# CityU-AIM-Group/SCAN

Hardware: AMD Instinct MI355X
Metric: train images/sec (whole node), VGG16 C2F 1024x2048 (higher is better)
Workload: dtype f32 (fp32 storage, fp32 multiply, fp32 accumulate -- the reference's arithmetic; the convolutions run it on the bf16 matrix cores as bf16x6: every fp32 operand cut into 3 bf16 pieces = all 24 significand bits, 6 bf16 MFMAs per product)

## Files before the change

scan_amd/csrc/capi.cpp:

```cpp
#include <stdarg.h>
#include <stdio.h>
#include <string.h>

#include "../../include/scan_hip.h"
#include "conv_launch.h"

static thread_local char g_err[512] = "";

extern "C" void scan_set_error(const char* fmt, ...) {
  va_list ap;
  va_start(ap, fmt);
  vsnprintf(g_err, sizeof(g_err), fmt, ap);
  va_end(ap);
}

extern "C" const char* scan_last_error(void) { return g_err; }
extern "C" int scan_abi_version(void) { return 1; }

int g_scan_deterministic = 0;

struct Knob {
  const char* key;
  int* slot;
  int dflt;
};
static Knob* knob_table(int* count) {
  static Knob knobs[] = {
      {"conv_bn256", &g_scan_conv_bn256, 0},   {"conv_v2", &g_scan_conv_v2, 0},         {"conv_wg1024", &g_scan_conv_wg1024, 0},
      {"conv_w8", &g_scan_conv_w8, 0},         {"conv_tpb3", &g_scan_conv_tpb3, 0},     {"conv_bn64_th16", &g_scan_conv_bn64_th16, 0},
      {"conv_glds", &g_scan_conv_glds, 0},     {"wgrad_v6", &g_scan_wgrad_v6, 0},       {"wgrad_prio", &g_scan_wgrad_prio, 0},
      {"wgrad_tile", &g_scan_wgrad_tile, 0},   {"wgrad_wgs", &g_scan_wgrad_wgs, 0},     {"gconv_mfma", &g_scan_gconv_mfma, 0},
      {"dbscan_bf16x3", &g_scan_dbscan_bf16x3, 0}, {"reduce_blocks", &g_scan_reduce_blocks, 0}, {"conv1x1", &g_scan_conv1x1, 0},
      {"conv_wino", &g_scan_conv_wino, 0},     {"wgrad_wino", &g_scan_wgrad_wino, 0},   {"wino_tpb", &g_scan_wino_tpb, 0},
      {"deterministic", &g_scan_deterministic, 0}, {"dynconv_generic", &g_scan_dynconv_generic, 0},
  };
  static bool init = false;
  if (!init) {
    for (auto& k : knobs) k.dflt = *k.slot;
    init = true;
  }
  *count = (int)(sizeof(knobs) / sizeof(knobs[0]));
  return knobs;
}
static Knob* find_knob(const char* key) {
  int n = 0;
  Knob* t = knob_table(&n);
  if (key == nullptr) return nullptr;
  for (int i = 0; i < n; ++i)
    if (strcmp(key, t[i].key) == 0) return &t[i];
  return nullptr;
}

extern "C" int scan_tune(const char* key, int value) {
  Knob* k = find_knob(key);
  if (k == nullptr) return SCAN_TUNE_UNKNOWN;
  const int old = *k->slot;
  *k->slot = value;
  return old;
}

extern "C" int scan_tune_get(const char* key) {
  const Knob* k = find_knob(key);
  return k == nullptr ? SCAN_TUNE_UNKNOWN : *k->slot;
}

extern "C" int scan_tune_default(const char* key) {
  const Knob* k = find_knob(key);
  return k == nullptr ? SCAN_TUNE_UNKNOWN : k->dflt;
}

extern "C" const char* scan_tune_key(int index) {
  int n = 0;
  const Knob* t = knob_table(&n);
  return (index >= 0 && index < n) ? t[index].key : nullptr;
}
```

scan_amd/csrc/conv_launch.h:

```cpp
#pragma once
#include <hip/hip_runtime_api.h>
#include <stdint.h>

#include "../../include/scan_hip.h"

extern int g_scan_conv_v2;
extern int g_scan_conv_bn256, g_scan_conv_wg1024, g_scan_conv_w8, g_scan_conv_tpb3;
extern int g_scan_conv_glds, g_scan_conv_bn64_th16, g_scan_conv1x1;
extern int g_scan_conv_wino, g_scan_wino_tpb;
extern int g_scan_wgrad_v6, g_scan_wgrad_prio, g_scan_wgrad_tile, g_scan_wgrad_wgs, g_scan_wgrad_wino;
extern int g_scan_gconv_mfma;
extern int g_scan_dynconv_generic;
extern int g_scan_dbscan_bf16x3;
extern int g_scan_reduce_blocks;

struct ConvArgs {
  const float* x;
  const scan_pyramid_t* od;
  const scan_pyramid_t* sd;
  int32_t Cs;
  const __bf16* w[3];
  int32_t Csw;
  const float* bias;
  const float* mask;
  float* y;
  int32_t Nout, Ns, relu, map;
  hipStream_t st;
  double* gn_ws;
};

struct ConvInst {
  int id;
  void (*launch)(const ConvArgs&);
};
ConvInst pick3x3(int np, const scan_pyramid_t* d, int32_t Nout, bool whole_chunks);
ConvInst pick1x1(int np, const scan_pyramid_t* yd, int32_t Nout, int32_t Csw);
void conv3x3_wino_launch(const ConvArgs& a);

void gen1_conv3x3_launch(const ConvArgs& a);
void gen1_conv1x1_launch(const ConvArgs& a);

typedef scan_conv_wgrad_plan_t WgradPlan;
int wgrad_split_plan(const char* name, int np, int ksize, int stride, int32_t Cs, int32_t Cout, const scan_pyramid_t* d, WgradPlan* p);
int wgrad_split_run(const char* name, const WgradPlan& p, const float* x, const scan_pyramid_t* xd, int32_t Cs, const float* dy,
                    const scan_pyramid_t* yd, int32_t Cout, int32_t Cout_s, float* dw, float* db, int32_t accumulate, float* ws,
                    void* stream);
int wgrad_generic_plan(const char* name, int np, int ksize, int stride, int32_t Cs, int32_t Cout, const scan_pyramid_t* yd, WgradPlan* p);
int wgrad_generic_run(const char* name, const WgradPlan& p, const float* x, const scan_pyramid_t* xd, int32_t Cs, const float* dy,
                      const scan_pyramid_t* yd, int32_t Cout, int32_t Cout_s, float* dw, float* db, int32_t accumulate, float* ws,
                      void* stream);
```

scan_amd/csrc/gconv.hip:

```cpp
#include "common.h"

#define GC_G 128

template <int CTRL, int ROW_MASK>
__device__ __forceinline__ float dpp_add(float v) {
  const int r = __builtin_amdgcn_update_dpp(0, __builtin_bit_cast(int, v), CTRL, ROW_MASK, 0xF, false);
  return v + __builtin_bit_cast(float, r);
}
__device__ __forceinline__ float half_wave_sum_hi(float v) {
  v = dpp_add<0xB1, 0xF>(v);
  v = dpp_add<0x4E, 0xF>(v);
  v = dpp_add<0x141, 0xF>(v);
  v = dpp_add<0x140, 0xF>(v);
  v = dpp_add<0x142, 0xA>(v);
  return v;
}

__device__ __forceinline__ int64_t neighbour_row(const scan_pyramid_t& d, int64_t m, const RowCoord& rc, int oy, int ox) {
  const int y = rc.y + oy, x = rc.x + ox;
  if (y < 0 || y >= d.h[rc.lvl] || x < 0 || x >= d.w[rc.lvl]) return -1;
  return m + (int64_t)oy * d.w[rc.lvl] + ox;
}

__device__ __forceinline__ float4 zero4() { return make_float4(0.f, 0.f, 0.f, 0.f); }
// ... 237 lines not shown
    wv[t] = DO_DX ? *reinterpret_cast<const float4*>(w + ((int64_t)g * 9 + t) * GC + coff) : zero4();
    acc[t] = zero4();
  }
  const bool need_x = DO_DW || relu_mask;
  constexpr int UN = (DO_DX && DO_DW) ? 1 : GC_UNROLL;
  for (int64_t q0 = hw / G; q0 < M; q0 += UN * J) {
    float4 h[UN];
    float gy[UN][9];
#pragma unroll
    for (int u = 0; u < UN; ++u) {
      const int64_t q = q0 + u * J;
      h[u] = (q < M && need_x) ? *reinterpret_cast<const float4*>(x + q * GC + coff) : zero4();
      if (q < M) {
        const RowCoord rc = decode_row(d, q);
#pragma unroll
        for (int t = 0; t < 9; ++t) {
          const int64_t p = neighbour_row(d, q, rc, 1 - t / 3, 1 - t % 3);
          gy[u][t] = p >= 0 ? dy[p * Ns + g] : 0.f;
        }
      } else {
#pragma unroll
        for (int t = 0; t < 9; ++t) gy[u][t] = 0.f;
      }
    }
#pragma unroll
    for (int u = 0; u < UN; ++u) {
      const int64_t q = q0 + u * J;
      if (DO_DW) {
#pragma unroll
        for (int t = 0; t < 9; ++t) fma4(acc[t], gy[u][t], h[u]);
      }
      if (DO_DX && q < M) {
        float4 o = zero4();
#pragma unroll
        for (int t = 0; t < 9; ++t) fma4(o, gy[u][t], wv[t]);
        if (relu_mask) o = relu_mask4(h[u], o);
        *reinterpret_cast<float4*>(dx + q * GC + coff) = o;
      }
    }
  }
  if (!DO_DW) return;
  float* out = slab + (int64_t)hw * 9 * GC_G + 4 * l32;
#pragma unroll
  for (int t = 0; t < 9; ++t) *reinterpret_cast<float4*>(out + t * GC_G) = acc[t];
}

typedef float f32x4g __attribute__((ext_vector_type(4)));

__global__ __launch_bounds__(256) void gconv_taps_mfma_kernel(const float* __restrict__ x, int64_t M, int G, int GC,
                                                              const float* __restrict__ w, float* __restrict__ T,
                                                              uint32_t* __restrict__ relu_bits) {
  const int lane = threadIdx.x & 63;
  const int col = lane & 15, q = lane >> 4;
  const int64_t wave_id = (int64_t)blockIdx.x * 4 + (threadIdx.x >> 6);
  const int64_t n_waves = (int64_t)gridDim.x * 4;
  const int g = (int)(wave_id % G);
  float4 bw[8];
#pragma unroll
  for (int j = 0; j < 8; ++j)
    bw[j] = col < 9 ? *reinterpret_cast<const float4*>(w + ((int64_t)g * 9 + col) * GC + g * GC_G + 16 * j + 4 * q)
                    : make_float4(0.f, 0.f, 0.f, 0.f);
  const int64_t groups = (M + 15) / 16;
  for (int64_t gidx = wave_id / G; gidx < groups; gidx += n_waves / G) {
    const int64_t row = gidx * 16 + col;
    float4 av[8];
#pragma unroll
    for (int j = 0; j < 8; ++j)
      av[j] = row < M ? *reinterpret_cast<const float4*>(x + row * GC + g * GC_G + 16 * j + 4 * q)
                      : make_float4(0.f, 0.f, 0.f, 0.f);
    f32x4g acc = {0.f, 0.f, 0.f, 0.f};
    uint32_t bits = 0u;
#pragma unroll
    for (int j = 0; j < 8; ++j) {
      acc = __builtin_amdgcn_mfma_f32_16x16x4f32(av[j].x, bw[j].x, acc, 0, 0, 0);
      acc = __builtin_amdgcn_mfma_f32_16x16x4f32(av[j].y, bw[j].y, acc, 0, 0, 0);
      acc = __builtin_amdgcn_mfma_f32_16x16x4f32(av[j].z, bw[j].z, acc, 0, 0, 0);
      acc = __builtin_amdgcn_mfma_f32_16x16x4f32(av[j].w, bw[j].w, acc, 0, 0, 0);
      bits |= (av[j].x > 0.f ? 1u : 0u) << (4 * j) | (av[j].y > 0.f ? 2u : 0u) << (4 * j) |
              (av[j].z > 0.f ? 4u : 0u) << (4 * j) | (av[j].w > 0.f ? 8u : 0u) << (4 * j);
    }
    if (relu_bits != nullptr && row < M) relu_bits[(row * G + g) * 4 + q] = bits;
#pragma unroll
    for (int r = 0; r < 4; ++r) {
      const int64_t orow = gidx * 16 + 4 * q + r;
      if (col < 9 && orow < M) T[(orow * G + g) * 9 + col] = acc[r];
    }
  }
}

__global__ __launch_bounds__(256) void gconv_dx_mfma_kernel(const float* __restrict__ dy, int Ns, scan_pyramid_t d, int G,
                                                            int GC, const float* __restrict__ w,
                                                            const float* __restrict__ xmask,
                                                            const uint32_t* __restrict__ relu_bits,
                                                            float* __restrict__ dx) {
  const int64_t M = d.row_off[d.n_levels];
  const int lane = threadIdx.x & 63;
  const int col = lane & 15, q = lane >> 4;
  const int64_t wave_id = (int64_t)blockIdx.x * 4 + (threadIdx.x >> 6);
  const int64_t n_waves = (int64_t)gridDim.x * 4;
  const int g = (int)(wave_id % G);
  float aw[8][3];
#pragma unroll
  for (int tile = 0; tile < 8; ++tile)
#pragma unroll
    for (int s_ = 0; s_ < 3; ++s_) {
      const int t = 4 * s_ + q;
      aw[tile][s_] = t < 9 ? w[((int64_t)g * 9 + t) * GC + g * GC_G + 16 * tile + col] : 0.f;
    }
  const int64_t groups = (M + 15) / 16;
  for (int64_t gidx = wave_id / G; gidx < groups; gidx += n_waves / G) {
    const int64_t row = gidx * 16 + col;
    float gy[3] = {0.f, 0.f, 0.f};
    if (row < M) {
      const RowCoord rc = decode_row(d, row);
#pragma unroll
      for (int s_ = 0; s_ < 3; ++s_) {
        const int t = 4 * s_ + q;
        if (t < 9) {
          const int64_t p = neighbour_row(d, row, rc, 1 - t / 3, 1 - t % 3);
          if (p >= 0) gy[s_] = dy[p * Ns + g];
        }
      }
    }
    uint32_t bits = 0xffffffffu;
    float4 mk[8];
    if (relu_bits != nullptr) {
      if (row < M) bits = relu_bits[(row * G + g) * 4 + q];
    } else if (xmask != nullptr) {
#pragma unroll
      for (int tile = 0; tile < 8; ++tile)
        mk[tile] = row < M ? *reinterpret_cast<const float4*>(xmask + row * GC + g * GC_G + 16 * tile + 4 * q)
                           : make_float4(0.f, 0.f, 0.f, 0.f);
    }
#pragma unroll
    for (int tile = 0; tile < 8; ++tile) {
      f32x4g acc = {0.f, 0.f, 0.f, 0.f};
#pragma unroll
      for (int s_ = 0; s_ < 3; ++s_) acc = __builtin_amdgcn_mfma_f32_16x16x4f32(aw[tile][s_], gy[s_], acc, 0, 0, 0);
      float4 o = make_float4(acc[0], acc[1], acc[2], acc[3]);
      if (relu_bits != nullptr) {
        o.x = (bits >> (4 * tile + 0)) & 1u ? o.x : 0.f;
        o.y = (bits >> (4 * tile + 1)) & 1u ? o.y : 0.f;
        o.z = (bits >> (4 * tile + 2)) & 1u ? o.z : 0.f;
        o.w = (bits >> (4 * tile + 3)) & 1u ? o.w : 0.f;
      } else if (xmask != nullptr) {
        o = relu_mask4(mk[tile], o);
      }
      if (row < M) *reinterpret_cast<float4*>(dx + row * GC + g * GC_G + 16 * tile + 4 * q) = o;
    }
  }
}

__global__ __launch_bounds__(256) void gconv_slab_partial_kernel(const float* __restrict__ slab, int blocks, int n,
                                                                 int per_part, float* __restrict__ partial) {
  const int i = blockIdx.x * blockDim.x + threadIdx.x;
  if (i >= n) return;
  const int b0 = blockIdx.y * per_part;
  const int b1 = b0 + per_part < blocks ? b0 + per_part : blocks;
  float s = 0.f;
#pragma unroll 8
  for (int b = b0; b < b1; ++b) s += slab[(int64_t)b * n + i];
  partial[(int64_t)blockIdx.y * n + i] = s;
}

enum GconvDst {
  GC_DST_DW,
  GC_DST_DW_GENERIC,
  GC_DST_DE
};
template <GconvDst DST>
__device__ __forceinline__ int64_t gconv_dst_index(int i, int GC) {
  if (DST == GC_DST_DW_GENERIC) {
    const int gt = i / GC_G, c = i - gt * GC_G;
    return (int64_t)gt * GC + (gt / 9) * GC_G + c;
  }
  const int t = i / GC, c = i - t * GC;
  return DST == GC_DST_DW ? ((int64_t)(c / GC_G) * 9 + t) * GC + c : ((int64_t)(c / GC_G) * 9 + t) * GC_G + c % GC_G;
}

template <GconvDst DST>
__global__ __launch_bounds__(256) void gconv_reduce_kernel(const float* __restrict__ partial, int parts, int GC,
                                                           float* __restrict__ out, int accumulate) {
  const int i = blockIdx.x * blockDim.x + threadIdx.x;
  if (i >= 9 * GC) return;
  float s = 0.f;
  for (int b = 0; b < parts; ++b) s += partial[(int64_t)b * 9 * GC + i];
  float* dst = out + gconv_dst_index<DST>(i, GC);
  *dst = accumulate ? *dst + s : s;
}


__device__ __forceinline__ float4 act_hidden(float4 h, const float4 (&ev)[9], const float (&av)[9]) {
#pragma unroll
  for (int t = 0; t < 9; ++t) fma4(h, av[t], ev[t]);
  return relu_mask4(h, h);
}

#define GC_UNROLL_A 2
#define GC_PICK_UNI(G, kernel, ...) ((G) == 8 ? kernel<true, ##__VA_ARGS__> : kernel<false, ##__VA_ARGS__>)

template <bool UNI>
__global__ __launch_bounds__(256) void gconv_taps_act_kernel(const float* __restrict__ x, scan_pyramid_t d, int G, int GC,
                                                             const float* __restrict__ w, const float* __restrict__ a,
                                                             int lda, const float* __restrict__ E, float* __restrict__ T) {
  const int64_t M = d.row_off[d.n_levels];
  const int quads = GC >> 2, slots = 256 / quads;
  const int cq = threadIdx.x % quads, slot = threadIdx.x / quads;
  const int g = cq >> 5, l32 = cq & 31;
  float4 wv[9], ev[9];
#pragma unroll
  for (int t = 0; t < 9; ++t) {
    wv[t] = *reinterpret_cast<const float4*>(w + ((int64_t)g * 9 + t) * GC + 4 * cq);
    ev[t] = *reinterpret_cast<const float4*>(E + ((int64_t)g * 9 + t) * GC_G + 4 * l32);
  }
  const int64_t stride = (int64_t)gridDim.x * slots;
  for (int64_t q0 = (int64_t)blockIdx.x * slots + slot; q0 < M; q0 += GC_UNROLL_F * stride) {
    float4 h[GC_UNROLL_F];
#pragma unroll
    for (int u = 0; u < GC_UNROLL_F; ++u) {
      const int64_t q = q0 + u * stride;
      h[u] = q < M ? *reinterpret_cast<const float4*>(x + q * GC + 4 * cq) : zero4();
    }
#pragma unroll
    for (int u = 0; u < GC_UNROLL_F; ++u) {
      int64_t q = q0 + u * stride;
      if (UNI) q = uniform_row(q);
      if (q >= M) continue;
      float av[9];
      tap_values<1>(d, q, decode_row(d, q), a, lda, g, UNI, av);
      tap_store(T, q, G, g, l32, tap_sums(act_hidden(h[u], ev, av), wv, l32));
    }
  }
}

template <bool UNI, bool FUSE>
__global__ __launch_bounds__(256, (UNI && !FUSE) ? 3 : 2) void gconv_bwd_act_kernel(
    const float* __restrict__ x, const float* __restrict__ dy, int Ns, scan_pyramid_t d, int G, int GC,
    const float* __restrict__ w, const float* __restrict__ a, int lda, const float* __restrict__ E, float* __restrict__ dx,
    float* __restrict__ slab, float* __restrict__ T, float* __restrict__ slab_e) {
  __shared__ float red[9 * 1024];
  const int64_t M = d.row_off[d.n_levels];
  const int quads = GC >> 2, slots = 256 / quads;
  const int cq = threadIdx.x % quads, slot = threadIdx.x / quads;
  const int g = cq >> 5, l32 = cq & 31;
  float4 wv[9], ev[9], acc[9], acc_e[9];
#pragma unroll
  for (int t = 0; t < 9; ++t) {
    wv[t] = *reinterpret_cast<const float4*>(w + ((int64_t)g * 9 + t) * GC + 4 * cq);
    ev[t] = *reinterpret_cast<const float4*>(E + ((int64_t)g * 9 + t) * GC_G + 4 * l32);
    acc[t] = zero4();
    if (FUSE) acc_e[t] = zero4();
  }
  for (int64_t q0 = (int64_t)blockIdx.x * GC_UNROLL_A * slots + slot; q0 < M;
       q0 += (int64_t)gridDim.x * GC_UNROLL_A * slots) {
    float4 h[GC_UNROLL_A];
#pragma unroll
    for (int u = 0; u < GC_UNROLL_A; ++u) {
      const int64_t q = q0 + u * slots;
      h[u] = q < M ? *reinterpret_cast<const float4*>(x + q * GC + 4 * cq) : zero4();
    }
#pragma unroll
    for (int u = 0; u < GC_UNROLL_A; ++u) {
      int64_t q = q0 + u * slots;
      if (UNI) q = uniform_row(q);
      if (q >= M) continue;
      const RowCoord rc = decode_row(d, q);
      float av[9], gy[9];
      tap_values<1>(d, q, rc, a, lda, g, UNI, av);
      const float4 hv = act_hidden(h[u], ev, av);
      tap_values<-1>(d, q, rc, dy, Ns, g, UNI, gy);
      float4 o = zero4();
#pragma unroll
      for (int t = 0; t < 9; ++t) {
        fma4(acc[t], gy[t], hv);
        fma4(o, gy[t], wv[t]);
      }
      o = relu_mask4(hv, o);
      *reinterpret_cast<float4*>(dx + q * GC + 4 * cq) = o;
      if (FUSE) {
        float mine = 0.f;
#pragma unroll
        for (int t = 0; t < 9; ++t) {
          fma4(acc_e[t], av[t], o);
          const float s = half_wave_sum_hi(dot4(o, ev[8 - t]));
          if (l32 == 16 + t) mine = s;
        }
        tap_store(T, q, G, g, l32, mine);
      }
    }
  }
  slab_store(acc, red, slab, GC);
  if (FUSE) {
    __syncthreads();
    slab_store(acc_e, red, slab_e, GC);
  }
}

template <bool UNI>
__global__ __launch_bounds__(256) void gconv_act_grads_kernel(const float* __restrict__ dh, scan_pyramid_t d, int G, int GC,
                                                              const float* __restrict__ a, int lda,
                                                              const float* __restrict__ E, float* __restrict__ T,
                                                              float* __restrict__ slab) {
  __shared__ float red[9 * 1024];
  const int64_t M = d.row_off[d.n_levels];
  const int quads = GC >> 2, slots = 256 / quads;
  const int cq = threadIdx.x % quads, slot = threadIdx.x / quads;
  const int g = cq >> 5, l32 = cq & 31;
  float4 ev[9], acc[9];
#pragma unroll
  for (int t = 0; t < 9; ++t) {
    ev[t] = *reinterpret_cast<const float4*>(E + ((int64_t)g * 9 + t) * GC_G + 4 * l32);
    acc[t] = zero4();
  }
  for (int64_t q0 = (int64_t)blockIdx.x * GC_UNROLL_A * slots + slot; q0 < M;
       q0 += (int64_t)gridDim.x * GC_UNROLL_A * slots) {
    float4 h[GC_UNROLL_A];
#pragma unroll
    for (int u = 0; u < GC_UNROLL_A; ++u) {
      const int64_t q = q0 + u * slots;
      h[u] = q < M ? *reinterpret_cast<const float4*>(dh + q * GC + 4 * cq) : zero4();
    }
#pragma unroll
    for (int u = 0; u < GC_UNROLL_A; ++u) {
      int64_t q = q0 + u * slots;
      if (UNI) q = uniform_row(q);
      if (q >= M) continue;
      float av[9];
      tap_values<1>(d, q, decode_row(d, q), a, lda, g, UNI, av);
      float mine = 0.f;
#pragma unroll
      for (int t = 0; t < 9; ++t) {
        fma4(acc[t], av[t], h[u]);
        const float s = half_wave_sum_hi(dot4(h[u], ev[8 - t]));
        if (l32 == 16 + t) mine = s;
      }
      tap_store(T, q, G, g, l32, mine);
    }
  }
  slab_store(acc, red, slab, GC);
}

#define GC_MAX_BLOCKS 1024
#define GC_PARTS 32
#define GC_GMAX 31

static bool gconv_lane_mapped(int G) { return G == 1 || G == 2 || G == 4 || G == 8; }

static int gconv_check(const scan_pyramid_t* d, int G, int Cg, const char* who, bool any_g = false) {
  SCAN_CHECK_ARG(d && d->n_levels >= 1 && d->n_levels <= SCAN_MAX_LEVELS, "%s: bad pyramid", who);
  SCAN_CHECK_ARG(Cg == GC_G, "%s: only 128 channels per group are built (got %d)", who, Cg);
  if (any_g) {
    SCAN_CHECK_ARG(G >= 1 && G <= GC_GMAX, "%s: G=%d out of 1..%d", who, G, GC_GMAX);
    return 0;
  }
  SCAN_CHECK_ARG(gconv_lane_mapped(G), "%s: G=%d must be 1, 2, 4 or 8", who, G);
  return 0;
}

int g_scan_gconv_mfma = 0;

enum GconvFamily { GC_GENERIC, GC_FMA, GC_MFMA };
static GconvFamily gconv_family(int G, bool bits) {
  if (!gconv_lane_mapped(G)) return GC_GENERIC;
  return (g_scan_gconv_mfma || bits) ? GC_MFMA : GC_FMA;
}

extern "C" int32_t scan_gconv3x3_to1_max_groups(void) { return GC_GMAX; }

extern "C" int32_t scan_gconv3x3_to1_caps(int32_t G, int32_t Cg) {
  if (G < 1 || G > GC_GMAX || Cg != GC_G) return 0;
  const GconvFamily f = gconv_family(G, false);
  return SCAN_GCONV_RUNS | (f == GC_GENERIC ? 0 : SCAN_GCONV_LANE_MAPPED) | (f == GC_MFMA ? SCAN_GCONV_BITS : 0) |
         (f == GC_FMA ? SCAN_GCONV_ACT : 0);
}

struct GconvWs {
  int64_t slab, slab_e, total;
};
static GconvWs gconv_ws_layout(int64_t M, int G, int Cg, bool act) {
  const int64_t taps = M * G * 9, slab = (int64_t)(GC_MAX_BLOCKS + GC_PARTS) * 9 * G * Cg;
  if (act) return {taps, taps + slab, taps + 2 * slab};
  return {0, -1, taps > slab ? taps : slab};
}

extern "C" int64_t scan_gconv3x3_to1_ws_floats(const scan_pyramid_t* d, int32_t G, int32_t Cg) {
  return d ? gconv_ws_layout(d->row_off[d->n_levels], G, Cg, false).total : -1;
}

extern "C" int64_t scan_gconv3x3_to1_act_ws_floats(const scan_pyramid_t* d, int32_t G, int32_t Cg) {
  return d ? gconv_ws_layout(d->row_off[d->n_levels], G, Cg, true).total : -1;
}

static int gconv_generic_strides(int64_t M, int per, int max_j) {
  int64_t j = ((M + per - 1) / per + 7) / 8 * 8;
  if (j < 8) j = 8;
  if (j > max_j) j = max_j;
  return (int)j;
}

static int gconv_slab_blocks(int64_t M) {
  int64_t rpb = (M + GC_MAX_BLOCKS - 1) / GC_MAX_BLOCKS;
  if (rpb < 16) rpb = 16;
  return (int)((M + rpb - 1) / rpb);
}

static int gconv_wave_grid(int64_t M, int G) {
  int64_t tasks = ((M + 15) / 16) * G;
  int64_t blocks = (tasks + 3) / 4;
  if (blocks > 2048) blocks = 2048;
  if (blocks < 2) blocks = 2;
  return (int)((blocks + 1) / 2 * 2);
}

static int gconv_gather(const float* T, const scan_pyramid_t* d, int G, const float* bias, float* y, int ldy, int col0,
                        hipStream_t st) {
  const int64_t M = d->row_off[d->n_levels];
  hipLaunchKernelGGL(gconv_gather_kernel, dim3(grid_for(M * ldy, 256)), dim3(256), 0, st, T, *d, G, bias, y, ldy, col0);
  SCAN_LAUNCH_CHECK("gconv_gather");
  return 0;
}

template <GconvDst DST>
static int gconv_slab_to(float* slab, int blocks, int GC, float* out, int accumulate, hipStream_t st) {
  const int n = 9 * GC, per = (blocks + GC_PARTS - 1) / GC_PARTS, parts = (blocks + per - 1) / per;
  float* partial = slab + (int64_t)GC_MAX_BLOCKS * n;
  hipLaunchKernelGGL(gconv_slab_partial_kernel, dim3((n + 255) / 256, parts), dim3(256), 0, st, slab, blocks, n, per, partial);
  SCAN_LAUNCH_CHECK("gconv_slab_partial");
  hipLaunchKernelGGL(gconv_reduce_kernel<DST>, dim3((n + 255) / 256), dim3(256), 0, st, partial, parts, GC, out, accumulate);
  SCAN_LAUNCH_CHECK(DST == GC_DST_DE ? "gconv_act_reduce" : "gconv_wgrad_reduce");
  return 0;
}

static int gconv_forward(const float* x, const scan_pyramid_t* d, int G, int Cg, const float* w, const float* bias, float* y,
                         int Ns, float* ws, uint32_t* relu_bits, hipStream_t st, bool any_g = false) {
  if (gconv_check(d, G, Cg, "gconv3x3_to1_forward", any_g)) return -1;
  SCAN_CHECK_ARG(x && w && y && ws && Ns >= G, "gconv3x3_to1_forward: bad arguments (Ns=%d)", Ns);
  const int64_t M = d->row_off[d->n_levels];
  if (M == 0) return 0;
  const int GC = G * Cg;
  switch (gconv_family(G, relu_bits != nullptr)) {
    case GC_GENERIC:
      SCAN_CHECK_ARG(relu_bits == nullptr, "gconv3x3_to1_forward_bits: G=%d must be 1, 2, 4 or 8", G);
      hipLaunchKernelGGL(gconv_taps_generic_kernel, dim3(gconv_generic_strides(M, GC_UNROLL_F, 2048) / 8 * G), dim3(256), 0,
                         st, x, M, G, GC, w, ws);
      SCAN_LAUNCH_CHECK("gconv_taps_generic");
      break;
    case GC_MFMA:
      hipLaunchKernelGGL(gconv_taps_mfma_kernel, dim3(gconv_wave_grid(M, G)), dim3(256), 0, st, x, M, G, GC, w, ws, relu_bits);
      SCAN_LAUNCH_CHECK("gconv_taps");
      break;
    case GC_FMA: {
      const int slots = 256 / (GC / 4);
      hipLaunchKernelGGL(gconv_taps_kernel, dim3(grid_for((M + slots - 1) / slots, 1)), dim3(256), 0, st, x, M, G, GC, w, ws);
      SCAN_LAUNCH_CHECK("gconv_taps");
    }
  }
  return gconv_gather(ws, d, G, bias, y, Ns, 0, st);
}

template <bool DO_DX, bool DO_DW>
static void gconv_bwd_launch(bool generic, int grid, hipStream_t st, const float* x, const float* dy, int Ns,
                             const scan_pyramid_t* d, int G, int GC, const float* w, int relu_mask, float* dx, float* slab) {
  hipLaunchKernelGGL((generic ? gconv_bwd_generic_kernel<DO_DX, DO_DW> : gconv_bwd_kernel<DO_DX, DO_DW>), dim3(grid), dim3(256),
                     0, st, x, dy, Ns, *d, G, GC, w, relu_mask, dx, slab);
}

static int gconv_backward(const float* x, const float* dy, int Ns, const scan_pyramid_t* d, int G, int Cg, const float* w,
                          int relu_mask, const uint32_t* relu_bits, float* dx, float* dw, int accumulate, float* ws,
                          hipStream_t st, const char* who, bool any_g = false) {
  if (gconv_check(d, G, Cg, who, any_g)) return -1;
  SCAN_CHECK_ARG(dy && Ns >= G && (dx || dw), "%s: bad arguments (Ns=%d)", who, Ns);
  SCAN_CHECK_ARG(!dx || w, "%s: the data gradient needs the weights", who);
  SCAN_CHECK_ARG(!dw || (x && ws), "%s: the weight gradient needs x and a workspace", who);
  SCAN_CHECK_ARG(!(dx && relu_mask && !relu_bits) || x, "%s: the ReLU mask needs x or its bit mask", who);
  const int64_t M = d->row_off[d->n_levels];
  if (M == 0) return 0;
  const int GC = G * Cg;
  const GconvFamily family = gconv_family(G, relu_bits != nullptr);
  const bool generic = family == GC_GENERIC;
  SCAN_CHECK_ARG(!generic || relu_bits == nullptr, "%s: G=%d must be 1, 2, 4 or 8", who, G);
  const int blocks = generic ? gconv_generic_strides(M, 16, GC_MAX_BLOCKS) : gconv_slab_blocks(M);
  const int grid = generic ? blocks / 8 * G : blocks;
  float* slab = ws + gconv_ws_layout(M, G, Cg, false).slab;
  if (dx && family == GC_MFMA) {
    hipLaunchKernelGGL(gconv_dx_mfma_kernel, dim3(gconv_wave_grid(M, G)), dim3(256), 0, st, dy, Ns, *d, G, GC, w,
                       (relu_mask && !relu_bits) ? x : (const float*)nullptr, relu_bits, dx);
    SCAN_LAUNCH_CHECK(who);
    if (dw) gconv_bwd_launch<false, true>(generic, grid, st, x, dy, Ns, d, G, GC, w, 0, dx, slab);
  } else if (dx && dw) {
    gconv_bwd_launch<true, true>(generic, grid, st, x, dy, Ns, d, G, GC, w, relu_mask, dx, slab);
  } else if (dx) {
    gconv_bwd_launch<true, false>(generic, grid, st, x, dy, Ns, d, G, GC, w, relu_mask, dx, slab);
  } else {
    gconv_bwd_launch<false, true>(generic, grid, st, x, dy, Ns, d, G, GC, w, 0, dx, slab);
  }
  SCAN_LAUNCH_CHECK(who);
  if (!dw) return 0;
  return generic ? gconv_slab_to<GC_DST_DW_GENERIC>(slab, blocks, GC, dw, accumulate, st)
                 : gconv_slab_to<GC_DST_DW>(slab, blocks, GC, dw, accumulate, st);
}

extern "C" int scan_gconv3x3_to1_forward(const float* x, const scan_pyramid_t* d, int32_t G, int32_t Cg, const float* w,
                                         const float* bias, float* y, int32_t Ns, float* ws, void* stream) {
  return gconv_forward(x, d, G, Cg, w, bias, y, Ns, ws, nullptr, as_stream(stream));
}

extern "C" int scan_gconv3x3_to1_forward_bits(const float* x, const scan_pyramid_t* d, int32_t G, int32_t Cg,
                                              const float* w, const float* bias, float* y, int32_t Ns, float* ws,
                                              uint32_t* relu_bits, void* stream) {
  SCAN_CHECK_ARG(relu_bits, "gconv3x3_to1_forward_bits: null bit mask");
  return gconv_forward(x, d, G, Cg, w, bias, y, Ns, ws, relu_bits, as_stream(stream));
}

extern "C" int scan_gconv3x3_to1_dgrad(const float* dy, int32_t Ns, const scan_pyramid_t* d, int32_t G, int32_t Cg,
                                       const float* w, const float* mask, float* dx, void* stream) {
  SCAN_CHECK_ARG(dx, "gconv3x3_to1_dgrad: null output");
  return gconv_backward(mask, dy, Ns, d, G, Cg, w, mask != nullptr, nullptr, dx, nullptr, 0, nullptr, as_stream(stream),
                        "gconv3x3_to1_dgrad");
}

extern "C" int scan_gconv3x3_to1_wgrad(const float* x, const float* dy, int32_t Ns, const scan_pyramid_t* d, int32_t G,
                                       int32_t Cg, float* dw, int32_t accumulate, float* ws, void* stream) {
  SCAN_CHECK_ARG(dw, "gconv3x3_to1_wgrad: null output");
  return gconv_backward(x, dy, Ns, d, G, Cg, nullptr, 0, nullptr, nullptr, dw, accumulate, ws, as_stream(stream),
                        "gconv3x3_to1_wgrad");
}

extern "C" int scan_gconv3x3_to1_backward(const float* x, const float* dy, int32_t Ns, const scan_pyramid_t* d, int32_t G,
                                          int32_t Cg, const float* w, int32_t relu_mask, float* dx, float* dw,
                                          int32_t accumulate, float* ws, void* stream) {
  SCAN_CHECK_ARG(x && dx && dw, "gconv3x3_to1_backward: null pointer");
  return gconv_backward(x, dy, Ns, d, G, Cg, w, relu_mask, nullptr, dx, dw, accumulate, ws, as_stream(stream),
                        "gconv3x3_to1_backward");
}

extern "C" int scan_gconv3x3_to1_backward_bits(const float* x, const float* dy, int32_t Ns, const scan_pyramid_t* d,
                                               int32_t G, int32_t Cg, const float* w, const uint32_t* relu_bits, float* dx,
                                               float* dw, int32_t accumulate, float* ws, void* stream) {
  SCAN_CHECK_ARG(x && dx && dw && relu_bits, "gconv3x3_to1_backward_bits: null pointer");
  return gconv_backward(x, dy, Ns, d, G, Cg, w, 1, relu_bits, dx, dw, accumulate, ws, as_stream(stream),
                        "gconv3x3_to1_backward_bits");
}

extern "C" int scan_gconv3x3_to1_any_forward(const float* x, const scan_pyramid_t* d, int32_t G, int32_t Cg, const float* w,
                                             const float* bias, float* y, int32_t Ns, float* ws, void* stream) {
  return gconv_forward(x, d, G, Cg, w, bias, y, Ns, ws, nullptr, as_stream(stream), true);
}

extern "C" int scan_gconv3x3_to1_any_dgrad(const float* dy, int32_t Ns, const scan_pyramid_t* d, int32_t G, int32_t Cg,
                                           const float* w, const float* mask, float* dx, void* stream) {
  SCAN_CHECK_ARG(dx, "gconv3x3_to1_any_dgrad: null output");
  return gconv_backward(mask, dy, Ns, d, G, Cg, w, mask != nullptr, nullptr, dx, nullptr, 0, nullptr, as_stream(stream),
                        "gconv3x3_to1_any_dgrad", true);
}

extern "C" int scan_gconv3x3_to1_any_wgrad(const float* x, const float* dy, int32_t Ns, const scan_pyramid_t* d, int32_t G,
                                           int32_t Cg, float* dw, int32_t accumulate, float* ws, void* stream) {
  SCAN_CHECK_ARG(dw, "gconv3x3_to1_any_wgrad: null output");
  return gconv_backward(x, dy, Ns, d, G, Cg, nullptr, 0, nullptr, nullptr, dw, accumulate, ws, as_stream(stream),
                        "gconv3x3_to1_any_wgrad", true);
}

extern "C" int scan_gconv3x3_to1_any_backward(const float* x, const float* dy, int32_t Ns, const scan_pyramid_t* d, int32_t G,
                                              int32_t Cg, const float* w, int32_t relu_mask, float* dx, float* dw,
                                              int32_t accumulate, float* ws, void* stream) {
  SCAN_CHECK_ARG(x && dx && dw, "gconv3x3_to1_any_backward: null pointer");
  return gconv_backward(x, dy, Ns, d, G, Cg, w, relu_mask, nullptr, dx, dw, accumulate, ws, as_stream(stream),
                        "gconv3x3_to1_any_backward", true);
}

static int gconv_act_check(const scan_pyramid_t* d, int G, int Cg, const float* a, int lda, int a_col0, const float* E,
                           const char* who) {
  if (gconv_check(d, G, Cg, who)) return -1;
  SCAN_CHECK_ARG(a && E && a_col0 >= 0 && lda >= a_col0 + G, "%s: bad act map (lda=%d, first column %d, G=%d)", who, lda,
                 a_col0, G);
  return 0;
}

extern "C" int scan_gconv3x3_to1_act_forward(const float* x, const scan_pyramid_t* d, int32_t G, int32_t Cg, const float* w,
                                             const float* bias, const float* a, int32_t lda, int32_t a_col0, const float* E,
                                             float* y, int32_t Ns, float* ws, void* stream) {
  if (gconv_act_check(d, G, Cg, a, lda, a_col0, E, "gconv3x3_to1_act_forward")) return -1;
  SCAN_CHECK_ARG(x && w && y && ws && Ns >= G, "gconv3x3_to1_act_forward: bad arguments (Ns=%d)", Ns);
  const int64_t M = d->row_off[d->n_levels];
  if (M == 0) return 0;
  const int GC = G * Cg, slots = 256 / (GC / 4);
  hipStream_t st = as_stream(stream);
  hipLaunchKernelGGL(GC_PICK_UNI(G, gconv_taps_act_kernel), dim3(grid_for((M + slots - 1) / slots, 1)), dim3(256), 0, st, x, *d,
                     G, GC, w, a + a_col0, lda, E, ws);
  SCAN_LAUNCH_CHECK("gconv_taps_act");
  return gconv_gather(ws, d, G, bias, y, Ns, 0, st);
}

extern "C" int scan_gconv3x3_to1_act_backward(const float* x, const float* dy, int32_t Ns, const scan_pyramid_t* d, int32_t G,
                                              int32_t Cg, const float* w, const float* a, int32_t lda, int32_t a_col0,
                                              const float* E, float* dx, float* dw, int32_t accumulate, float* ws,
                                              void* stream) {
  if (gconv_act_check(d, G, Cg, a, lda, a_col0, E, "gconv3x3_to1_act_backward")) return -1;
  SCAN_CHECK_ARG(x && dy && w && dx && dw && ws && Ns >= G, "gconv3x3_to1_act_backward: bad arguments (Ns=%d)", Ns);
  const int64_t M = d->row_off[d->n_levels];
  if (M == 0) return 0;
  const int GC = G * Cg, blocks = gconv_slab_blocks(M);
  hipStream_t st = as_stream(stream);
  float* slab = ws + gconv_ws_layout(M, G, Cg, true).slab;
  hipLaunchKernelGGL(GC_PICK_UNI(G, gconv_bwd_act_kernel, false), dim3(blocks), dim3(256), 0, st, x, dy, Ns, *d, G, GC, w,
                     a + a_col0, lda, E, dx, slab, (float*)nullptr, (float*)nullptr);
  SCAN_LAUNCH_CHECK("gconv_bwd_act");
  return gconv_slab_to<GC_DST_DW>(slab, blocks, GC, dw, accumulate, st);
}

extern "C" int scan_gconv3x3_to1_act_grads(const float* dh, const scan_pyramid_t* d, int32_t G, int32_t Cg, const float* a,
                                           int32_t lda, int32_t a_col0, const float* E, float* da, int32_t ldda,
                                           int32_t da_col0, float* dE, int32_t accumulate, float* ws, void* stream) {
  if (gconv_act_check(d, G, Cg, a, lda, a_col0, E, "gconv3x3_to1_act_grads")) return -1;
  SCAN_CHECK_ARG(dh && da && dE && ws && da_col0 >= 0 && ldda >= da_col0 + G,
                 "gconv3x3_to1_act_grads: bad arguments (ldda=%d, first column %d)", ldda, da_col0);
  const int64_t M = d->row_off[d->n_levels];
  if (M == 0) return 0;
  const int GC = G * Cg, blocks = gconv_slab_blocks(M);
  hipStream_t st = as_stream(stream);
  float* slab = ws + gconv_ws_layout(M, G, Cg, true).slab;
  hipLaunchKernelGGL(GC_PICK_UNI(G, gconv_act_grads_kernel), dim3(blocks), dim3(256), 0, st, dh, *d, G, GC, a + a_col0, lda, E,
                     ws, slab);
  SCAN_LAUNCH_CHECK("gconv_act_grads");
  if (int rc = gconv_gather(ws, d, G, nullptr, da, ldda, da_col0, st)) return rc;
  return gconv_slab_to<GC_DST_DE>(slab, blocks, GC, dE, accumulate, st);
}

extern "C" int scan_gconv3x3_to1_act_backward_all(const float* x, const float* dy, int32_t Ns, const scan_pyramid_t* d,
                                                  int32_t G, int32_t Cg, const float* w, const float* a, int32_t lda,
                                                  int32_t a_col0, const float* E, float* dx, float* dw, float* da, int32_t ldda,
                                                  int32_t da_col0, float* dE, int32_t accumulate, float* ws, void* stream) {
  if (gconv_act_check(d, G, Cg, a, lda, a_col0, E, "gconv3x3_to1_act_backward_all")) return -1;
  SCAN_CHECK_ARG(x && dy && w && dx && dw && ws && Ns >= G, "gconv3x3_to1_act_backward_all: bad arguments (Ns=%d)", Ns);
  SCAN_CHECK_ARG(da && dE && da_col0 >= 0 && ldda >= da_col0 + G,
                 "gconv3x3_to1_act_backward_all: bad arguments (ldda=%d, first column %d)", ldda, da_col0);
  const int64_t M = d->row_off[d->n_levels];
  if (M == 0) return 0;
  const int GC = G * Cg, blocks = gconv_slab_blocks(M);
  hipStream_t st = as_stream(stream);
  const GconvWs L = gconv_ws_layout(M, G, Cg, true);
  hipLaunchKernelGGL(GC_PICK_UNI(G, gconv_bwd_act_kernel, true), dim3(blocks), dim3(256), 0, st, x, dy, Ns, *d, G, GC, w,
                     a + a_col0, lda, E, dx, ws + L.slab, ws, ws + L.slab_e);
  SCAN_LAUNCH_CHECK("gconv_bwd_act");
  if (int rc = gconv_gather(ws, d, G, nullptr, da, ldda, da_col0, st)) return rc;
  if (int rc = gconv_slab_to<GC_DST_DW>(ws + L.slab, blocks, GC, dw, accumulate, st)) return rc;
  return gconv_slab_to<GC_DST_DE>(ws + L.slab_e, blocks, GC, dE, accumulate, st);
}
```

Before: 25.53.

## Add software-pipelined gconv activation kernels and batch the dw/dE slab reductions

```diff
diff --git a/scan_amd/csrc/capi.cpp b/scan_amd/csrc/capi.cpp
--- a/scan_amd/csrc/capi.cpp
+++ b/scan_amd/csrc/capi.cpp
@@ -33,6 +33,7 @@
       {"dbscan_bf16x3", &g_scan_dbscan_bf16x3, 0}, {"reduce_blocks", &g_scan_reduce_blocks, 0}, {"conv1x1", &g_scan_conv1x1, 0},
       {"conv_wino", &g_scan_conv_wino, 0},     {"wgrad_wino", &g_scan_wgrad_wino, 0},   {"wino_tpb", &g_scan_wino_tpb, 0},
       {"deterministic", &g_scan_deterministic, 0}, {"dynconv_generic", &g_scan_dynconv_generic, 0},
+      {"gconv_pipe", &g_scan_gconv_pipe, 0},
   };
   static bool init = false;
   if (!init) {
diff --git a/scan_amd/csrc/conv_launch.h b/scan_amd/csrc/conv_launch.h
--- a/scan_amd/csrc/conv_launch.h
+++ b/scan_amd/csrc/conv_launch.h
@@ -10,6 +10,7 @@
 extern int g_scan_conv_wino, g_scan_wino_tpb;
 extern int g_scan_wgrad_v6, g_scan_wgrad_prio, g_scan_wgrad_tile, g_scan_wgrad_wgs, g_scan_wgrad_wino;
 extern int g_scan_gconv_mfma;
+extern int g_scan_gconv_pipe;
 extern int g_scan_dynconv_generic;
 extern int g_scan_dbscan_bf16x3;
 extern int g_scan_reduce_blocks;
diff --git a/scan_amd/csrc/gconv.hip b/scan_amd/csrc/gconv.hip
--- a/scan_amd/csrc/gconv.hip
+++ b/scan_amd/csrc/gconv.hip
@@ -413,9 +413,12 @@
 }
 
 __global__ __launch_bounds__(256) void gconv_slab_partial_kernel(const float* __restrict__ slab, int blocks, int n,
-                                                                 int per_part, float* __restrict__ partial) {
+                                                                 int per_part, float* __restrict__ partial,
+                                                                 int64_t z_stride) {
   const int i = blockIdx.x * blockDim.x + threadIdx.x;
   if (i >= n) return;
+  slab += blockIdx.z * z_stride;
+  partial += blockIdx.z * z_stride;
   const int b0 = blockIdx.y * per_part;
   const int b1 = b0 + per_part < blocks ? b0 + per_part : blocks;
   float s = 0.f;
@@ -447,6 +450,18 @@
   float s = 0.f;
   for (int b = 0; b < parts; ++b) s += partial[(int64_t)b * 9 * GC + i];
   float* dst = out + gconv_dst_index<DST>(i, GC);
+  *dst = accumulate ? *dst + s : s;
+}
+
+__global__ __launch_bounds__(256) void gconv_reduce_pair_kernel(const float* __restrict__ partial, int64_t z_stride, int parts,
+                                                                int GC, float* __restrict__ dw, float* __restrict__ dE,
+                                                                int accumulate) {
+  const int i = blockIdx.x * blockDim.x + threadIdx.x;
+  if (i >= 9 * GC) return;
+  partial += blockIdx.y * z_stride;
+  float s = 0.f;
+  for (int b = 0; b < parts; ++b) s += partial[(int64_t)b * 9 * GC + i];
+  float* dst = blockIdx.y == 0 ? dw + gconv_dst_index<GC_DST_DW>(i, GC) : dE + gconv_dst_index<GC_DST_DE>(i, GC);
   *dst = accumulate ? *dst + s : s;
 }
 
@@ -601,6 +616,294 @@
   slab_store(acc, red, slab, GC);
 }
 
+#define GC_PIPE_ROWS 4
+
+typedef float f32x4p __attribute__((ext_vector_type(4)));
+
+#define GC_PIPE_PHASE() __builtin_amdgcn_sched_barrier(0)
+#define GC_PIPE_TAP(fine, t) do { if ((fine) && (t) % 3 == 2 && (t) < 8) GC_PIPE_PHASE(); } while (0)
+
+__device__ __forceinline__ float4 lds_quad(const float4* img, int t, int off) { return img[t * 256 + off]; }
+
+struct RowGather {
+  const float* src;
+  int ld, oy, ox;
+  int put;
+  int get;
+};
+__device__ __forceinline__ RowGather row_gather(const float* __restrict__ a, int lda, const float* __restrict__ dy, int Ns) {
+  const int l = threadIdx.x & 63, i = l & 31, half = l >> 5;
+  const int g0 = 2 * (int)(threadIdx.x >> 6), tl = i % 9, gl = i / 9;
+  const bool on = i < 18 && (half == 0 || dy != nullptr);
+  RowGather rg;
+  rg.src = on ? (half ? dy : a) + g0 + gl : nullptr;
+  rg.ld = half ? Ns : lda;
+  rg.oy = half ? 1 - tl / 3 : tl / 3 - 1;
+  rg.ox = half ? 1 - tl % 3 : tl % 3 - 1;
+  rg.put = on ? 32 * half + 12 * gl + tl : -1;
+  rg.get = 12 * half;
+  return rg;
+}
+__device__ __forceinline__ float row_gather_load(const scan_pyramid_t& d, int64_t q, const RowGather& rg) {
+  const RowCoord rc = decode_row(d, q);
+  const int64_t p = rg.src != nullptr ? neighbour_row(d, q, rc, rg.oy, rg.ox) : -1;
+  return p >= 0 ? rg.src[p * rg.ld] : 0.f;
+}
+__device__ __forceinline__ void row_gather_put(float* win, const RowGather& rg, float val) {
+  __builtin_amdgcn_fence(__ATOMIC_RELEASE, "wavefront");
+  __builtin_amdgcn_wave_barrier();
+  if (rg.put >= 0) win[rg.put] = val;
+  __builtin_amdgcn_fence(__ATOMIC_RELEASE, "wavefront");
+  __builtin_amdgcn_wave_barrier();
+  __builtin_amdgcn_fence(__ATOMIC_ACQUIRE, "wavefront");
+}
+__device__ __forceinline__ void row_gather_get(const float* win, int at, float (&v)[9]) {
+  const f32x4p lo = *reinterpret_cast<const f32x4p*>(win + at), hi = *reinterpret_cast<const f32x4p*>(win + at + 4);
+  v[0] = lo[0], v[1] = lo[1], v[2] = lo[2], v[3] = lo[3];
+  v[4] = hi[0], v[5] = hi[1], v[6] = hi[2], v[7] = hi[3];
+  v[8] = win[at + 8];
+}
+
+template <bool UNI>
+__global__ __launch_bounds__(256, 4) void gconv_taps_act_pipe_kernel(const float* __restrict__ x, scan_pyramid_t d, int G,
+                                                                     int GC, const float* __restrict__ w,
+                                                                     const float* __restrict__ a, int lda,
+                                                                     const float* __restrict__ E, float* __restrict__ T) {
+  __shared__ __attribute__((aligned(16))) float4 le[9 * 256];
+  __shared__ __attribute__((aligned(16))) float window[UNI ? 256 : 4];
+  constexpr int R = GC_PIPE_ROWS;
+  const int64_t M = d.row_off[d.n_levels];
+  const int quads = GC >> 2, slots = 256 / quads;
+  const int cq = threadIdx.x % quads, slot = threadIdx.x / quads;
+  const int g = cq >> 5, l32 = cq & 31;
+  float4 wv[9];
+#pragma unroll
+  for (int t = 0; t < 9; ++t) {
+    wv[t] = *reinterpret_cast<const float4*>(w + ((int64_t)g * 9 + t) * GC + 4 * cq);
+    le[t * 256 + threadIdx.x] = *reinterpret_cast<const float4*>(E + ((int64_t)g * 9 + t) * GC_G + 4 * l32);
+  }
+  const RowGather rg = row_gather(a, lda, nullptr, 0);
+  float* win = window + (UNI ? 64 * (threadIdx.x >> 6) : 0);
+  const int64_t stride = (int64_t)gridDim.x * slots, first = (int64_t)blockIdx.x * slots + slot;
+  float4 hn[R];
+  float tn[R];
+#pragma unroll
+  for (int u = 0; u < R; ++u) {
+    int64_t q = first + u * stride;
+    if (UNI) q = uniform_row(q);
+    hn[u] = q < M ? *reinterpret_cast<const float4*>(x + q * GC + 4 * cq) : zero4();
+    tn[u] = (UNI && q < M) ? row_gather_load(d, q, rg) : 0.f;
+  }
+  for (int64_t q0 = first; q0 < M; q0 += R * stride) {
+    float4 h[R];
+    float tv[R];
+#pragma unroll
+    for (int u = 0; u < R; ++u) {
+      h[u] = hn[u], tv[u] = tn[u];
+      int64_t q = q0 + (R + u) * stride;
+      if (UNI) q = uniform_row(q);
+      hn[u] = q < M ? *reinterpret_cast<const float4*>(x + q * GC + 4 * cq) : zero4();
+      tn[u] = (UNI && q < M) ? row_gather_load(d, q, rg) : 0.f;
+    }
+#pragma unroll
+    for (int u = 0; u < R; ++u) {
+      int64_t q = q0 + u * stride;
+      if (UNI) q = uniform_row(q);
+      if (q >= M) continue;
+      int off = threadIdx.x;
+      asm volatile("" : "+v"(off));
+      GC_PIPE_PHASE();
+      float av[9];
+      if (UNI) {
+        row_gather_put(win, rg, tv[u]);
+        row_gather_get(win, rg.get, av);
+      } else {
+        tap_values<1>(d, q, decode_row(d, q), a, lda, g, false, av);
+      }
+      float4 hv = h[u];
+#pragma unroll
+      for (int t = 0; t < 9; ++t) {
+        fma4(hv, av[t], lds_quad(le, t, off));
+        GC_PIPE_TAP(true, t);
+      }
+      hv = relu_mask4(hv, hv);
+      GC_PIPE_PHASE();
+      tap_store(T, q, G, g, l32, tap_sums(hv, wv, l32));
+    }
+  }
+}
+
+template <bool UNI, bool FUSE>
+__global__ __launch_bounds__(256, FUSE ? 2 : 3) void gconv_bwd_act_pipe_kernel(
+    const float* __restrict__ x, const float* __restrict__ dy, int Ns, scan_pyramid_t d, int G, int GC,
+    const float* __restrict__ w, const float* __restrict__ a, int lda, const float* __restrict__ E, float* __restrict__ dx,
+    float* __restrict__ slab, float* __restrict__ T, float* __restrict__ slab_e) {
+  __shared__ __attribute__((aligned(16))) float4 le[9 * 256];
+  __shared__ __attribute__((aligned(16))) float4 lw[FUSE ? 9 * 256 : 1];
+  __shared__ __attribute__((aligned(16))) float window[UNI ? 256 : 4];
+  constexpr int UA = GC_UNROLL_A, R = FUSE ? GC_PIPE_ROWS : UA;
+  const int64_t M = d.row_off[d.n_levels];
+  const int quads = GC >> 2, slots = 256 / quads;
+  const int cq = threadIdx.x % quads, slot = threadIdx.x / quads;
+  const int g = cq >> 5, l32 = cq & 31;
+  float4 wv[9], acc[9], acc_e[9];
+#pragma unroll
+  for (int t = 0; t < 9; ++t) {
+    wv[t] = *reinterpret_cast<const float4*>(w + ((int64_t)g * 9 + t) * GC + 4 * cq);
+    if (FUSE) lw[t * 256 + threadIdx.x] = wv[t];
+    le[t * 256 + threadIdx.x] = *reinterpret_cast<const float4*>(E + ((int64_t)g * 9 + t) * GC_G + 4 * l32);
+    acc[t] = zero4();
+    if (FUSE) acc_e[t] = zero4();
+  }
+  const RowGather rg = row_gather(a, lda, dy, Ns);
+  float* win = window + (UNI ? 64 * (threadIdx.x >> 6) : 0);
+  const int64_t first = (int64_t)blockIdx.x * UA * slots + slot, step = (int64_t)gridDim.x * UA * slots;
+  float4 hn[R];
+  float tn[R];
+#pragma unroll
+  for (int u = 0; u < R; ++u) {
+    int64_t q = first + (u / UA) * step + (u % UA) * slots;
+    if (UNI) q = uniform_row(q);
+    hn[u] = q < M ? *reinterpret_cast<const float4*>(x + q * GC + 4 * cq) : zero4();
+    tn[u] = (UNI && q < M) ? row_gather_load(d, q, rg) : 0.f;
+  }
+  for (int64_t q0 = first; q0 < M; q0 += (R / UA) * step) {
+    float4 h[R];
+    float tv[R];
+#pragma unroll
+    for (int u = 0; u < R; ++u) {
+      h[u] = hn[u], tv[u] = tn[u];
+      int64_t q = q0 + (R / UA + u / UA) * step + (u % UA) * slots;
+      if (UNI) q = uniform_row(q);
+      hn[u] = q < M ? *reinterpret_cast<const float4*>(x + q * GC + 4 * cq) : zero4();
+      tn[u] = (UNI && q < M) ? row_gather_load(d, q, rg) : 0.f;
+    }
+#pragma unroll
+    for (int u = 0; u < R; ++u) {
+      int64_t q = q0 + (u / UA) * step + (u % UA) * slots;
+      if (UNI) q = uniform_row(q);
+      if (q >= M) continue;
+      int off = threadIdx.x;
+      asm volatile("" : "+v"(off));
+      GC_PIPE_PHASE();
+      float av[9], gy[9];
+      if (UNI) {
+        row_gather_put(win, rg, tv[u]);
+        row_gather_get(win, rg.get, av);
+        row_gather_get(win, 32 + rg.get, gy);
+      } else {
+        const RowCoord rc = decode_row(d, q);
+        tap_values<1>(d, q, rc, a, lda, g, false, av);
+        tap_values<-1>(d, q, rc, dy, Ns, g, false, gy);
+      }
+      float4 hv = h[u];
+#pragma unroll
+      for (int t = 0; t < 9; ++t) {
+        fma4(hv, av[t], lds_quad(le, t, off));
+        GC_PIPE_TAP(!FUSE, t);
+      }
+      hv = relu_mask4(hv, hv);
+      GC_PIPE_PHASE();
+      float4 o = zero4();
+#pragma unroll
+      for (int t = 0; t < 9; ++t) {
+        fma4(acc[t], gy[t], hv);
+        fma4(o, gy[t], FUSE ? lds_quad(lw, t, off) : wv[t]);
+        GC_PIPE_TAP(!FUSE, t);
+      }
+      o = relu_mask4(hv, o);
+      *reinterpret_cast<float4*>(dx + q * GC + 4 * cq) = o;
+      if (FUSE) {
+        GC_PIPE_PHASE();
+        float mine = 0.f;
+#pragma unroll
+        for (int t = 0; t < 9; ++t) {
+          fma4(acc_e[t], av[t], o);
+          const float s = half_wave_sum_hi(dot4(o, lds_quad(le, 8 - t, off)));
+          if (l32 == 16 + t) mine = s;
+        }
+        tap_store(T, q, G, g, l32, mine);
+      }
+    }
+  }
+  float* red = reinterpret_cast<float*>(le);
+  slab_store(acc, red, slab, GC);
+  if (FUSE) {
+    __syncthreads();
+    slab_store(acc_e, red, slab_e, GC);
+  }
+}
+
+template <bool UNI>
+__global__ __launch_bounds__(256, 4) void gconv_act_grads_pipe_kernel(const float* __restrict__ dh, scan_pyramid_t d, int G,
+                                                                      int GC, const float* __restrict__ a, int lda,
+                                                                      const float* __restrict__ E, float* __restrict__ T,
+                                                                      float* __restrict__ slab) {
+  __shared__ __attribute__((aligned(16))) float4 le[9 * 256];
+  __shared__ __attribute__((aligned(16))) float window[UNI ? 256 : 4];
+  constexpr int UA = GC_UNROLL_A, R = UA;
+  const int64_t M = d.row_off[d.n_levels];
+  const int quads = GC >> 2, slots = 256 / quads;
+  const int cq = threadIdx.x % quads, slot = threadIdx.x / quads;
+  const int g = cq >> 5, l32 = cq & 31;
+  float4 acc[9];
+#pragma unroll
+  for (int t = 0; t < 9; ++t) {
+    le[t * 256 + threadIdx.x] = *reinterpret_cast<const float4*>(E + ((int64_t)g * 9 + t) * GC_G + 4 * l32);
+    acc[t] = zero4();
+  }
+  const RowGather rg = row_gather(a, lda, nullptr, 0);
+  float* win = window + (UNI ? 64 * (threadIdx.x >> 6) : 0);
+  const int64_t first = (int64_t)blockIdx.x * UA * slots + slot, step = (int64_t)gridDim.x * UA * slots;
+  float4 hn[R];
+  float tn[R];
+#pragma unroll
+  for (int u = 0; u < R; ++u) {
+    int64_t q = first + (u / UA) * step + (u % UA) * slots;
+    if (UNI) q = uniform_row(q);
+    hn[u] = q < M ? *reinterpret_cast<const float4*>(dh + q * GC + 4 * cq) : zero4();
+    tn[u] = (UNI && q < M) ? row_gather_load(d, q, rg) : 0.f;
+  }
+  for (int64_t q0 = first; q0 < M; q0 += (R / UA) * step) {
+    float4 h[R];
+    float tv[R];
+#pragma unroll
+    for (int u = 0; u < R; ++u) {
+      h[u] = hn[u], tv[u] = tn[u];
+      int64_t q = q0 + (R / UA + u / UA) * step + (u % UA) * slots;
+      if (UNI) q = uniform_row(q);
+      hn[u] = q < M ? *reinterpret_cast<const float4*>(dh + q * GC + 4 * cq) : zero4();
+      tn[u] = (UNI && q < M) ? row_gather_load(d, q, rg) : 0.f;
+    }
+#pragma unroll
+    for (int u = 0; u < R; ++u) {
+      int64_t q = q0 + (u / UA) * step + (u % UA) * slots;
+      if (UNI) q = uniform_row(q);
+      if (q >= M) continue;
+      int off = threadIdx.x;
+      asm volatile("" : "+v"(off));
+      GC_PIPE_PHASE();
+      float av[9];
+      if (UNI) {
+        row_gather_put(win, rg, tv[u]);
+        row_gather_get(win, rg.get, av);
+      } else {
+        tap_values<1>(d, q, decode_row(d, q), a, lda, g, false, av);
+      }
+      float mine = 0.f;
+#pragma unroll
+      for (int t = 0; t < 9; ++t) {
+        fma4(acc[t], av[t], h[u]);
+        const float s = half_wave_sum_hi(dot4(h[u], lds_quad(le, 8 - t, off)));
+        if (l32 == 16 + t) mine = s;
+        GC_PIPE_TAP(true, t);
+      }
+      tap_store(T, q, G, g, l32, mine);
+    }
+  }
+  slab_store(acc, reinterpret_cast<float*>(le), slab, GC);
+}
+
 #define GC_MAX_BLOCKS 1024
 #define GC_PARTS 32
 #define GC_GMAX 31
@@ -619,6 +922,8 @@
 }
 
 int g_scan_gconv_mfma = 0;
+
+int g_scan_gconv_pipe = 1;
 
 enum GconvFamily { GC_GENERIC, GC_FMA, GC_MFMA };
 static GconvFamily gconv_family(int G, bool bits) {
@@ -685,10 +990,24 @@
 static int gconv_slab_to(float* slab, int blocks, int GC, float* out, int accumulate, hipStream_t st) {
   const int n = 9 * GC, per = (blocks + GC_PARTS - 1) / GC_PARTS, parts = (blocks + per - 1) / per;
   float* partial = slab + (int64_t)GC_MAX_BLOCKS * n;
-  hipLaunchKernelGGL(gconv_slab_partial_kernel, dim3((n + 255) / 256, parts), dim3(256), 0, st, slab, blocks, n, per, partial);
+  hipLaunchKernelGGL(gconv_slab_partial_kernel, dim3((n + 255) / 256, parts), dim3(256), 0, st, slab, blocks, n, per, partial,
+                     (int64_t)0);
   SCAN_LAUNCH_CHECK("gconv_slab_partial");
   hipLaunchKernelGGL(gconv_reduce_kernel<DST>, dim3((n + 255) / 256), dim3(256), 0, st, partial, parts, GC, out, accumulate);
   SCAN_LAUNCH_CHECK(DST == GC_DST_DE ? "gconv_act_reduce" : "gconv_wgrad_reduce");
+  return 0;
+}
+
+static int gconv_slab_pair_to(float* slab, int64_t z_stride, int blocks, int GC, float* dw, float* dE, int accumulate,
+                              hipStream_t st) {
+  const int n = 9 * GC, per = (blocks + GC_PARTS - 1) / GC_PARTS, parts = (blocks + per - 1) / per;
+  float* partial = slab + (int64_t)GC_MAX_BLOCKS * n;
+  hipLaunchKernelGGL(gconv_slab_partial_kernel, dim3((n + 255) / 256, parts, 2), dim3(256), 0, st, slab, blocks, n, per, partial,
+                     z_stride);
+  SCAN_LAUNCH_CHECK("gconv_slab_partial");
+  hipLaunchKernelGGL(gconv_reduce_pair_kernel, dim3((n + 255) / 256, 2), dim3(256), 0, st, partial, z_stride, parts, GC, dw, dE,
+                     accumulate);
+  SCAN_LAUNCH_CHECK("gconv_reduce_pair");
   return 0;
 }
 
@@ -847,8 +1166,8 @@
   if (M == 0) return 0;
   const int GC = G * Cg, slots = 256 / (GC / 4);
   hipStream_t st = as_stream(stream);
-  hipLaunchKernelGGL(GC_PICK_UNI(G, gconv_taps_act_kernel), dim3(grid_for((M + slots - 1) / slots, 1)), dim3(256), 0, st, x, *d,
-                     G, GC, w, a + a_col0, lda, E, ws);
+  hipLaunchKernelGGL((g_scan_gconv_pipe ? GC_PICK_UNI(G, gconv_taps_act_pipe_kernel) : GC_PICK_UNI(G, gconv_taps_act_kernel)),
+                     dim3(grid_for((M + slots - 1) / slots, 1)), dim3(256), 0, st, x, *d, G, GC, w, a + a_col0, lda, E, ws);
   SCAN_LAUNCH_CHECK("gconv_taps_act");
   return gconv_gather(ws, d, G, bias, y, Ns, 0, st);
 }
@@ -864,8 +1183,9 @@
   const int GC = G * Cg, blocks = gconv_slab_blocks(M);
   hipStream_t st = as_stream(stream);
   float* slab = ws + gconv_ws_layout(M, G, Cg, true).slab;
-  hipLaunchKernelGGL(GC_PICK_UNI(G, gconv_bwd_act_kernel, false), dim3(blocks), dim3(256), 0, st, x, dy, Ns, *d, G, GC, w,
-                     a + a_col0, lda, E, dx, slab, (float*)nullptr, (float*)nullptr);
+  hipLaunchKernelGGL(
+      (g_scan_gconv_pipe ? GC_PICK_UNI(G, gconv_bwd_act_pipe_kernel, false) : GC_PICK_UNI(G, gconv_bwd_act_kernel, false)),
+      dim3(blocks), dim3(256), 0, st, x, dy, Ns, *d, G, GC, w, a + a_col0, lda, E, dx, slab, (float*)nullptr, (float*)nullptr);
   SCAN_LAUNCH_CHECK("gconv_bwd_act");
   return gconv_slab_to<GC_DST_DW>(slab, blocks, GC, dw, accumulate, st);
 }
@@ -881,8 +1201,8 @@
   const int GC = G * Cg, blocks = gconv_slab_blocks(M);
   hipStream_t st = as_stream(stream);
   float* slab = ws + gconv_ws_layout(M, G, Cg, true).slab;
-  hipLaunchKernelGGL(GC_PICK_UNI(G, gconv_act_grads_kernel), dim3(blocks), dim3(256), 0, st, dh, *d, G, GC, a + a_col0, lda, E,
-                     ws, slab);
+  hipLaunchKernelGGL((g_scan_gconv_pipe ? GC_PICK_UNI(G, gconv_act_grads_pipe_kernel) : GC_PICK_UNI(G, gconv_act_grads_kernel)),
+                     dim3(blocks), dim3(256), 0, st, dh, *d, G, GC, a + a_col0, lda, E, ws, slab);
   SCAN_LAUNCH_CHECK("gconv_act_grads");
   if (int rc = gconv_gather(ws, d, G, nullptr, da, ldda, da_col0, st)) return rc;
   return gconv_slab_to<GC_DST_DE>(slab, blocks, GC, dE, accumulate, st);
@@ -901,10 +1221,12 @@
   const int GC = G * Cg, blocks = gconv_slab_blocks(M);
   hipStream_t st = as_stream(stream);
   const GconvWs L = gconv_ws_layout(M, G, Cg, true);
-  hipLaunchKernelGGL(GC_PICK_UNI(G, gconv_bwd_act_kernel, true), dim3(blocks), dim3(256), 0, st, x, dy, Ns, *d, G, GC, w,
-                     a + a_col0, lda, E, dx, ws + L.slab, ws, ws + L.slab_e);
+  hipLaunchKernelGGL(
+      (g_scan_gconv_pipe ? GC_PICK_UNI(G, gconv_bwd_act_pipe_kernel, true) : GC_PICK_UNI(G, gconv_bwd_act_kernel, true)),
+      dim3(blocks), dim3(256), 0, st, x, dy, Ns, *d, G, GC, w, a + a_col0, lda, E, dx, ws + L.slab, ws, ws + L.slab_e);
   SCAN_LAUNCH_CHECK("gconv_bwd_act");
   if (int rc = gconv_gather(ws, d, G, nullptr, da, ldda, da_col0, st)) return rc;
+  if (g_scan_gconv_pipe) return gconv_slab_pair_to(ws + L.slab, L.slab_e - L.slab, blocks, GC, dw, dE, accumulate, st);
   if (int rc = gconv_slab_to<GC_DST_DW>(ws + L.slab, blocks, GC, dw, accumulate, st)) return rc;
   return gconv_slab_to<GC_DST_DE>(ws + L.slab_e, blocks, GC, dE, accumulate, st);
 }
```

Measured after the change: 25.60, median of 3. Within noise of the previous version (+0.3%).
